# aleflabo/HypAD

Hardware: AMD Instinct MI355X
Metric: training windows/sec (seq_len=100) (higher is better)
Workload: dtype f32; 1 GPU; configs[1]: univariate synthetic (sine+noise+jump), hyperbolic=True, batch=64, window=100, latent=20, 1916 windows/signal, 1 signal(s) per GPU; step = 1 epoch = 29 x (5 critic_x + 5 critic_z + 1 decoder) iterations; signals_per_gpu=1, launch=hipGraph replay of the captured epoch, rccl_world_size=1

## Files before the change

### hypad_amd/csrc/train_common.h

```cpp
#pragma once
#include <hip/hip_runtime.h>

#include "../../include/hypad.h"
#include "critic_valu.h"
#include "nets.h"

namespace hypad {
namespace train {

constexpr int THREADS = 256;
constexpr int TB = 512;

struct CritWs {
  int in_right, act[4], left[5], dm[4], partial, total;
};
HD CritWs crit_ws(int B, int in_dim, int L, int nh) {
  CritWs w; int o = 0;
  w.in_right = o; o += pad4(3 * B * in_dim);
  for (int i = 0; i < 4; ++i) { w.act[i] = o; if (i < nh) o += pad4(3 * B * L); }
  for (int i = 0; i < 5; ++i) { w.left[i] = o; if (i < nh) o += pad4(3 * B * L); else if (i == nh) o += pad4(3 * B); }
  for (int i = 0; i < 4; ++i) { w.dm[i] = o; if (i < nh) o += pad4(B * L); }
  w.partial = o; o += pad4((B / 16) * 4);
  w.total = o;
  return w;
}
struct GenWs {
  int xg, enc_g, enc_g2, enc_h, zcat, a0, g0, h0d, mask, g1, h1, ecat, u, du, ballpart, dpre2, dg1, dg0, da0, dzenc, dgenc, partial, adamc, total;
};
HD GenWs gen_ws(int B, int S, int L) {
  GenWs w; int o = 0;
  w.xg = o; o += pad4(2 * B * S);
  w.enc_g = o; o += pad4(B * 8 * ENC_H);
  w.enc_g2 = o; o += pad4(B * 8 * ENC_H);
  w.enc_h = o; o += pad4(2 * B * 2 * ENC_H);
  w.zcat = o; o += pad4(2 * B * L);
  w.a0 = o; o += pad4(2 * B * DEC_D1);
  w.g0 = o; o += pad4(2 * B * 8 * DEC_H);
  w.h0d = o; o += pad4(2 * B * 2 * DEC_H);
  w.mask = o; o += pad4(2 * B * 2 * DEC_H);
  w.g1 = o; o += pad4(2 * B * 8 * DEC_H);
  w.h1 = o; o += pad4(2 * B * 2 * DEC_H);
  w.ecat = o; o += pad4(3 * B * S);
  w.u = o; o += pad4(3 * B * S);
  w.du = o; o += pad4(3 * B * S);
  w.ballpart = o; o += pad4(2 * (B / 16) * S);
  w.dpre2 = o; o += pad4(2 * B * S);
  w.dg1 = o; o += pad4(2 * B * 6 * DEC_H);
  w.dg0 = o; o += pad4(2 * B * 6 * DEC_H);
  w.da0 = o; o += pad4(2 * B * DEC_D1);
  w.dzenc = o; o += pad4(2 * B * L);
  w.dgenc = o; o += pad4(2 * B * 6 * ENC_H);
  w.partial = o; o += pad4((B / 16) * 4);
  w.adamc = o; o += 4;
  w.total = o;
  return w;
}
inline int64_t ws_cz_offset(const hypad_dims& d) { return crit_ws(d.batch, d.signal_shape, d.latent_dim, 4).total; }
inline int64_t ws_pack_offset(const hypad_dims& d) {
  int64_t a = ws_cz_offset(d) + crit_ws(d.batch, d.latent_dim, d.latent_dim, 2).total;
  int64_t c = gen_ws(d.batch, d.signal_shape, d.latent_dim).total;
  return ((a > c ? a : c) + 63) & ~(int64_t)63;
}
constexpr int DW_ITEM_WORDS = 32, DW_ITEM_CAP = 2048;
inline int64_t ws_items_offset(const hypad_dims& d) {
  return (ws_pack_offset(d) + gen_pack(d.signal_shape, d.latent_dim, d.hyperbolic).total + 63) & ~(int64_t)63;
}
inline int64_t ws_floats_per_signal(const hypad_dims& d) {
  return ws_items_offset(d) + (int64_t)DW_ITEM_WORDS * DW_ITEM_CAP;
}

struct IterArgs {
  int S, L, B, hyperbolic;
  hypad_nets P, M, V;
  int pe, pd, pcx, pcz;
  int32_t* counters;
  const float* x; int64_t x_sig_stride; int64_t x_ld; const int32_t* row_index;
  const float* z; const float* alpha;
  int drop_mode;
  const float* masks; int64_t mask_sig_stride;
  uint64_t seed;
  float* losses; int64_t loss_sig_stride;
  float* ws; int64_t ws_sig_stride;
  int64_t pk_off;
  float lr, b1, b2, eps, wd; int stabilize; int riemannian;
  int opt;
  int tick_owner;
  int sig0;
  int step_add;
  int rng_sig0;
  int64_t ri_sig_stride;
  int guard;
  long long* stamps;
};
#if HYPAD_DIAG
#define GEN_STAMP(k) do { if (a.stamps && (threadIdx.x & 63) == 0 && blockIdx.x == 0 && blockIdx.y == 0) a.stamps[(blockIdx.z * 48 + (k)) * 8 + (threadIdx.x >> 6)] = (long long)__builtin_amdgcn_s_memtime(); } while (0)
#else
#define GEN_STAMP(k) do { } while (0)
#endif

struct LdsPlan {
  int xs, zs, bufA, bufB, crit, small, wst, cparams, total, ldS, bufFloats;
  int stage;
};
constexpr int LDS_LIMIT_FLOATS = 160 * 1024 / 4;
HD LdsPlan lds_plan(int S, int rows_lstm, int rows_head, int critic_floats, int crit_scratch = CRITIC_LDS_FLOATS) {
  LdsPlan p;
  p.ldS = lds_stride(S);
  int a = rows_lstm * (6 * DEC_H + 4), b = rows_head * p.ldS;
  p.bufFloats = a > b ? a : b;
  int o = 0;
  p.xs = o; o += 16 * p.ldS;
  p.zs = o; o += 32 * LP;
  p.bufA = o; o += p.bufFloats;
  p.bufB = o; o += p.bufFloats;
  p.crit = o; o += crit_scratch;
  p.small = o; o += 3 * 16 * LP + 64;
  p.wst = o; o += (TB / 64) * WSTAGE_FLOATS;
  p.cparams = o;
  p.stage = (o + critic_floats <= LDS_LIMIT_FLOATS) ? 1 : 0;
  if (p.stage) o += critic_floats;
  p.total = o;
  return p;
}

__device__ __forceinline__ DropSrc drop_src(const IterArgs& a, int sig, const float* ptr, uint32_t stream, uint32_t tick, float p) {
  DropSrc s;
  s.mode = a.drop_mode; s.ptr = ptr; s.batch = a.B; s.seed = a.seed; s.tick = tick; s.stream = stream; s.sig = (uint32_t)(sig + a.rng_sig0); s.p = p;
  return s;
// ... 101 lines not shown
```

### hypad_amd/csrc/train_iters.hip

```cpp
#include <hip/hip_runtime.h>

#include <cstdlib>
#include <type_traits>

#include <vector>

#include "../../include/hypad.h"
#include "critic_mfma.h"
#include "train_common.h"

using namespace hypad;
using namespace hypad::train;

namespace {

__device__ __forceinline__ void critic_three_passes(const IterArgs& a, int sig, int tile, uint32_t tick, const float* real, int ldr,
                                                    const float* fake, int ldf, float* inter, int ldi, float* gbuf, int ldgb,
                                                    const float* P, const CriticLayout& cl, const CriticBatchLds& cb, float* ws,
                                                    const CritWs& cw, int mask_real, int mask_fake, int mask_inter, float* red) {
  const int L = a.L, B = a.B, nh = cl.nh, in_dim = cl.in_dim, LQ = cb.LQ;
  const int g0 = tile * 16;
  const float* mbase = a.masks ? a.masks + sig * a.mask_sig_stride : nullptr;
  const int64_t mblk = (int64_t)nh * B * L;
  const int midx[3] = {mask_real, mask_fake, mask_inter};
// ... 194 lines not shown
  const int a = 16 * (6 * DEC_H + 4), b = rows_head * p.ldS;
  const int bufFloats = a > b ? a : b;
  int o = 0;
  p.hb = o; o += (role == 1 && hyper) ? 16 * p.ldS : 0;
  p.xs = o; o += role >= 1 ? 16 * p.ldS : 0;
  p.zs = o; o += 32 * LP;
  p.bufA = o; o += bufFloats;
  p.bufB = o; o += bufFloats;
  p.small = o; o += 3 * 16 * LP + 64;
  p.cw = o; o += cp.total;
  p.ct = o; o += critic_tile_floats(cp, role == 0 ? 4 : 2);
  p.total = o;
  return p;
}

template <int SC, int LC, int BC, bool WSC1 = false>
__device__ __forceinline__ void gen_role_z(const IterArgs& a, float* smem) {
  const int S = SC ? SC : a.S, L = LC ? LC : a.L, B = BC ? BC : a.B;
  const int sig = blockIdx.y + a.sig0, tile = blockIdx.x >> 3;
  const GenLds lp = gen_lds(S, L, a.hyperbolic, 2);
  const int ldS = lp.ldS;
  const GenWs gw = gen_ws(B, S, L);
  float* ws = a.ws + sig * a.ws_sig_stride;
  const float* pk = ws + a.pk_off;
  const GenPack gp = gen_pack(S, L, a.hyperbolic);
  float* xs = smem + lp.xs; float* zs = smem + lp.zs; float* bufA = smem + lp.bufA; float* bufB = smem + lp.bufB;
  float* dzc = smem + lp.small;
  float* cw = smem + lp.cw; float* ct = smem + lp.ct;
  const uint32_t tick = (uint32_t)a.counters[3] + (uint32_t)(a.step_add > 0 ? a.step_add : 0);
  const int g0 = tile * 16;
  const float* mbase = a.masks ? a.masks + sig * a.mask_sig_stride : nullptr;
  const CriticLayout clz = cz_layout(L);
  const CriticPad cpz = critic_pad(L, L, 2);
  tile_load_rows(xs, ldS, a.x + sig * a.x_sig_stride, a.x_ld, a.row_index ? a.row_index + (int64_t)sig * a.ri_sig_stride : nullptr, g0, 16, S, 16);
  const LstmPre pre_enc = lstm_layer_prefetch<WSC1>(pk + gp.enc_g[0], pk + gp.enc_g[1], ENC_H, S);
  stage_critic_padded(cw, a.P.cz + (int64_t)sig * a.pcz, clz, L, cpz);
  __syncthreads();
  tile_store(ws + gw.xg + (int64_t)(B + g0) * S, S, xs, ldS, 16, S, 16);
  float* zin = zs + 16 * LP;
  float* gates = ws + gw.enc_g2 + (int64_t)g0 * 8 * ENC_H;
  encoder_fwd_tile_packed<true, WSC1>(xs, ldS, S, L, pk, gp, bufA, ENC_LDG, bufB, ENC_LDH, zin, gates,
                                ws + gw.enc_h + (int64_t)(B + g0) * 2 * ENC_H, 16, pre_enc);
  const PackedPre pre_edt = gemm_nt_prefetch<WSC1>(pk + gp.enc_d_t, L, 2 * ENC_H);
  const DropSrc dz = drop_src(a, sig, mbase, RS_DROP_CRITIC + 8 * 0, tick, clz.p_drop);
  const float sum_crit = critic_tile_fwd_bwd(zin, LP, cw, clz, L, cpz, ct, -1.f / B, [&](int li, int r, int c) { return dz.get4(li, g0 + r, c, L); },
                                             [&](int li, int r, int c) { return dz.get(li, g0 + r, c, L); }, dzc, LP);
  tile_store(ws + gw.dzenc + (int64_t)(B + g0) * L, L, dzc, LP, 16, L, 16);
  float* dP = bufA;
  {
    LstmCellBwdEpi epi{gates, ENC_H, dP, ENC_LDG, 16, 16, nullptr, 0, ws + gw.dgenc + (int64_t)(B + g0) * 6 * ENC_H, {}, {}, {}, {}, {}};
    gemm_nt_packed_epi<1, true, decltype(epi), WSC1>(dzc, LP, L, 2 * ENC_H, pk + gp.enc_d_t, nullptr, 0, pre_edt, epi);
  }
  float* part_out = ws + gw.partial + tile * 4;
  if (threadIdx.x == 0) part_out[2] = sum_crit;
  if (tile == 0 && blockIdx.y == 0 && threadIdx.x == 0) {
    const int step = a.counters[a.opt] + 1 + (a.step_add > 0 ? a.step_add : 0);
    if (a.step_add < 0) a.counters[a.opt] = step;
    const AdamCoef c0 = adam_coef(a.lr, a.b1, a.b2, a.eps, a.wd, a.riemannian, a.stabilize, step);
    float* ac = a.ws + (int64_t)a.sig0 * a.ws_sig_stride + gw.adamc;
    ac[0] = c0.bc1; ac[1] = c0.bc2; ac[2] = c0.sqrt_bc2;
  }
}

static_assert(TB == 512, "gen_body deals rows over 8 waves");
template <bool HYPER, int SC, int LC, int BC, bool WSC1 = false>
__device__ __forceinline__ void gen_body(const IterArgs& a, float* smem) {
  const int S = SC ? SC : a.S, L = LC ? LC : a.L, B = BC ? BC : a.B;
  const int sig = blockIdx.y + a.sig0, tile = blockIdx.x >> 3, role = blockIdx.z;
  __builtin_amdgcn_s_setprio(2);
  if (role == 2) { gen_role_z<SC, LC, BC, WSC1>(a, smem); return; }
  const GenLds lp = gen_lds(S, L, HYPER ? 1 : 0, role);
  const int ldS = lp.ldS;
  const EncLayout el = enc_layout(S, L);
  const DecLayout dl = dec_layout(S, L, HYPER ? 1 : 0);
  const GenWs gw = gen_ws(B, S, L);
  const float* PE = a.P.enc + (int64_t)sig * a.pe;
  const float* PD = a.P.dec + (int64_t)sig * a.pd;
  float* ws = a.ws + sig * a.ws_sig_stride;
  const float* pk = ws + a.pk_off;
  const GenPack gp = gen_pack(S, L, HYPER ? 1 : 0);
  float* xs = smem + lp.xs; float* zs = smem + lp.zs; float* bufA = smem + lp.bufA; float* bufB = smem + lp.bufB;
  float* small = smem + lp.small;
  float* red = small + 3 * 16 * LP;
  float* cw = smem + lp.cw; float* ct = smem + lp.ct;
  float* Ein = (HYPER && role == 1) ? smem + lp.hb : bufA;
  const uint32_t tick = (uint32_t)a.counters[3] + (uint32_t)(a.step_add > 0 ? a.step_add : 0);
  const int g0 = tile * 16;
  const int pass = role;
  const int64_t prow0 = (int64_t)pass * B + g0;
  const float* mbase = a.masks ? a.masks + sig * a.mask_sig_stride : nullptr;
  const int64_t BL = (int64_t)B * L;
  const int lane = threadIdx.x & 63, wave = wave_id(), nw = blockDim.x >> 6;
  float sum_crit = 0.f, sum_aux = 0.f;
  constexpr int ldH = 2 * DEC_H + 4, ldG = 6 * DEC_H + 4, ldA0 = 52;
  GEN_STAMP(0);
  float* zin;
  PackedPre pre_d1;
  if (role == 0) {
    pre_d1 = gemm_nt_prefetch<WSC1>(pk + gp.d1, L, DEC_D1);
    const CriticLayout clx = cx_layout(S, L);
    stage_critic_padded(cw, a.P.cx + (int64_t)sig * a.pcx, clx, L, critic_pad(S, L, 4));
    load_z(a, sig, tile, tick, zs);
    zin = zs;
    __syncthreads();
  } else {
    GEN_STAMP(14);
    tile_load_rows(xs, ldS, a.x + sig * a.x_sig_stride, a.x_ld, a.row_index ? a.row_index + (int64_t)sig * a.ri_sig_stride : nullptr, g0, 16, S, 16);
    const LstmPre pre_enc = lstm_layer_prefetch<WSC1>(pk + gp.enc_g[0], pk + gp.enc_g[1], ENC_H, S);
    GEN_STAMP(15);
    GEN_STAMP(12);
    __syncthreads();
    GEN_STAMP(13);
    tile_store(ws + gw.xg + (int64_t)g0 * S, S, xs, ldS, 16, S, 16);
    if (HYPER) tile_store(ws + gw.ecat + (int64_t)(2 * B + g0) * S, S, xs, ldS, 16, S, 16);
    zin = zs + 16 * LP;
    encoder_fwd_tile_packed<true, WSC1>(xs, ldS, S, L, pk, gp, bufA, ENC_LDG, bufB, ENC_LDH, zin,
                                  ws + gw.enc_g + (int64_t)g0 * 8 * ENC_H, ws + gw.enc_h + (int64_t)g0 * 2 * ENC_H, 16, pre_enc);
    GEN_STAMP(1);
    pre_d1 = gemm_nt_prefetch<WSC1>(pk + gp.d1, L, DEC_D1);
  }
  GEN_STAMP(2);
  tile_store(ws + gw.zcat + prow0 * L, L, zin, LP, 16, L, 16);
  DecSave sv;
  sv.ps = 16;
  sv.a0 = ws + gw.a0 + prow0 * DEC_D1;
// ... 29 lines not shown
        for (int e = 0; e < EPL; ++e) { u_keep[e] = u.v[e]; hb_keep[e] = hb.v[e]; }
        row_store(bufB + r * ldS, head_row(u, hb), S, lane);
      }
    });
    __syncthreads();
  }
  float* R = HYPER ? bufB : bufA;
  float* dR = HYPER ? bufA : bufB;
  GEN_STAMP(4);
  if (role == 0) {
    const CriticLayout clx = cx_layout(S, L);
    const DropSrc dx = drop_src(a, sig, mbase ? mbase + 2 * BL : nullptr, RS_DROP_CRITIC + 8 * 1, tick, clx.p_drop);
    sum_crit = critic_tile_fwd_bwd(R, ldS, cw, clx, L, critic_pad(S, L, 4), ct, -1.f / B,
                                   [&](int li, int r, int c) { return dx.get4(li, g0 + r, c, L); },
                                   [&](int li, int r, int c) { return dx.get(li, g0 + r, c, L); }, dR, ldS);
  }
  GEN_STAMP(5);
  if (HYPER) {
    if (role == 1) {
      float part = 0.f;
      if (wave < 4) {
        epl16_dispatch(S, [&](auto tag) {
          using R16 = RowT<16, decltype(tag)::value>;
          const int r = wave * 4 + (lane >> 4);
          R16 du, dv;
          const float d = rowdist_row_bwd(row_load<R16>(R + r * ldS, S, lane), row_load<R16>(R + (16 + r) * ldS, S, lane), 10.f / B, du, dv);
          row_store(dR + r * ldS, du, S, lane);
          row_store(dR + (16 + r) * ldS, dv, S, lane);
          const float d0 = __int_as_float(__builtin_amdgcn_readlane(__float_as_int(d), 0)), d1 = __int_as_float(__builtin_amdgcn_readlane(__float_as_int(d), 16));
          const float d2 = __int_as_float(__builtin_amdgcn_readlane(__float_as_int(d), 32)), d3 = __int_as_float(__builtin_amdgcn_readlane(__float_as_int(d), 48));
          part = (d0 + d1) + (d2 + d3);
        });
      }
      if (lane == 0) red[16 + wave] = part;
      __syncthreads();
      for (int w = 0; w < nw; ++w) sum_aux += red[16 + w];
    }
    GEN_STAMP(23);
    const PackedPre pre_ht = gemm_nt_prefetch<WSC1>(pk + gp.head_t, S, S);
    epl16_dispatch(S, [&](auto tag) {
      constexpr int EPL = decltype(tag)::value;
      using R16 = RowT<16, EPL>;
      const int r = wave * 4 + (lane >> 4);
      if (wave * 4 < hrows) {
        R16 du, db, u, hb;
#pragma unroll
        for (int e = 0; e < EPL; ++e) { u.v[e] = u_keep[e]; hb.v[e] = hb_keep[e]; }
        head_row_bwd(u, hb, row_load<R16>(dR + r * ldS, S, lane), du, db);
        row_store(dR + r * ldS, du, S, lane);
        row_store(ws + gw.du + (prow0 + prow(r, B)) * S, du, S, lane);
#pragma unroll
        for (int e = 0; e < R16::EPL; ++e) {
          float v = db.v[e];
          v += __shfl_xor(v, 16, 64);
          v += __shfl_xor(v, 32, 64);
          db.v[e] = v;
        }
        if (lane < 16) row_store(R + wave * ldS, db, S, lane);
      }
    });
    __syncthreads();
    GEN_STAMP(24);
    for (int c = threadIdx.x; c < S; c += blockDim.x) {
      float s = 0.f;
      for (int w = 0; w < hrows / 4; ++w) s += R[w * ldS + c];
      ws[gw.ballpart + ((int64_t)role * (B / 16) + tile) * S + c] = s;
    }
    __syncthreads();
    GEN_STAMP(25);
    {
      struct TanhBwdEpi {
        float* Ys; int ldy; const float* E; int ldE; float* gout; float e[4]; int vo;
        __device__ __forceinline__ void prefetch(int n, int q, bool ok) {
          vo = (4 * q * ldE + (ok ? n : 0)) * 4;
          const GBuf eb(E);
#pragma unroll
          for (int r = 0; r < 4; ++r) e[r] = ok ? eb.ld(vo, r * ldE * 4) : 0.f;
        }
        __device__ __forceinline__ void emit(int, int r, int row, int n, float v) {
          const float o = v * (1.f - e[r] * e[r]);
          Ys[row * ldy + n] = o; GBuf(gout).st(o, vo, r * ldE * 4);
        }
      } epi{R, ldS, ws + gw.ecat + prow0 * S, S, ws + gw.dpre2 + prow0 * S, {}, 0};
      gemm_nt_packed_epi<1, true, decltype(epi), WSC1>(dR, ldS, S, S, pk + gp.head_t, nullptr, 0, pre_ht, epi);
    }
    __syncthreads();
    GEN_STAMP(26);
  } else {
    if (role == 1) {
      float part = 0.f;
      tile_for(16, S, [&](int r, int c) {
        const float diff = R[r * ldS + c] - xs[r * ldS + c];
        part += diff * diff;
        dR[r * ldS + c] = 20.f * diff / ((float)B * (float)S);
      });
      sum_aux = block_sum(part, red);
      __syncthreads();
    }
    tile_for(16, S, [&](int r, int c) {
      const float e = R[r * ldS + c];
      dR[r * ldS + c] *= 1.f - e * e;
// ... 20 lines not shown
    LstmCellBwdEpi epi{ws + gw.g0 + prow0 * 8 * DEC_H, DEC_H, X, ldG, 16, 16,
                       a.drop_mode != 0 ? ws + gw.mask + prow0 * 2 * DEC_H : nullptr, 2 * DEC_H, ws + gw.dg0 + prow0 * 6 * DEC_H, {}, {}, {}, {}, {}};
    gemm_nt_packed_epi<1, true, decltype(epi), WSC1>(Y, ldG, 6 * DEC_H, 2 * DEC_H, pk + gp.l_t[1], nullptr, 0, pre_l1t, epi);
  }
  GEN_STAMP(35);
  __syncthreads();
  GEN_STAMP(36);
  GEN_STAMP(8);
  GEN_STAMP(37);
  PackedPre pre_d1t{};
  if (role == 1) pre_d1t = gemm_nt_prefetch<WSC1>(pk + gp.d1_t, DEC_D1, L);
  GEN_STAMP(38);
  gemm_nt_packed<1, true, ActIdentity, WSC1>(X, ldG, 6 * DEC_H, DEC_D1, pk + gp.l_t[0], nullptr, Y, ldA0, 0, 0, pre_l0t, ActIdentity{}, nullptr, 0,
                          ws + gw.da0 + prow0 * DEC_D1, DEC_D1);
  GEN_STAMP(39);
  __syncthreads();
  GEN_STAMP(9);
  float* part_out = ws + gw.partial + tile * 4;
  if (role == 0) {
    if (threadIdx.x == 0) part_out[1] = sum_crit;
    GEN_STAMP(11);
    return;
  }
  const PackedPre pre_edt = gemm_nt_prefetch<WSC1>(pk + gp.enc_d_t, L, 2 * ENC_H);
  gemm_nt_packed<1, true, ActIdentity, WSC1>(Y, ldA0, DEC_D1, L, pk + gp.d1_t, nullptr, X, LP, 0, 0, pre_d1t, ActIdentity{}, nullptr, 0,
                          ws + gw.dzenc + (int64_t)g0 * L, L);
  __syncthreads();
  GEN_STAMP(10);
  {
    LstmCellBwdEpi epi{ws + gw.enc_g + (int64_t)g0 * 8 * ENC_H, ENC_H, Y, ENC_LDG, 16, 16, nullptr, 0,
                       ws + gw.dgenc + (int64_t)g0 * 6 * ENC_H, {}, {}, {}, {}, {}};
    gemm_nt_packed_epi<1, true, decltype(epi), WSC1>(X, LP, L, 2 * ENC_H, pk + gp.enc_d_t, nullptr, 0, pre_edt, epi);
  }
  if (threadIdx.x == 0) part_out[0] = sum_aux;
  GEN_STAMP(11);
}

__global__ __launch_bounds__(TB) void cx_pass_kernel(IterArgs a) {
  extern __shared__ __attribute__((aligned(16))) float smem[];
  cx_pass_body(a, smem);
}
__global__ __launch_bounds__(TB) void cz_pass_kernel(IterArgs a) {
  extern __shared__ __attribute__((aligned(16))) float smem[];
  cz_pass_body(a, smem);
}
__global__ __launch_bounds__(TB) void critic_pass_pair_kernel(IterArgs ax, IterArgs az) {
  extern __shared__ __attribute__((aligned(16))) float smem[];
  if (blockIdx.z == 0) cx_pass_body(ax, smem); else cz_pass_body(az, smem);
}
template <bool IS_X>
__global__ __launch_bounds__(TB) void critic_gp_kernel(IterArgs a) {
  extern __shared__ __attribute__((aligned(16))) float smem[];
  gp_body<IS_X>(a, smem);
}
__global__ __launch_bounds__(TB) void critic_gp_pair_kernel(IterArgs ax, IterArgs az) {
  extern __shared__ __attribute__((aligned(16))) float smem[];
  if (blockIdx.z == 0) gp_body<true>(ax, smem); else gp_body<false>(az, smem);
}
template <bool HYPER, int SC, int LC, int BC>
__global__ __launch_bounds__(TB) void gen_kernel(IterArgs a) {
  extern __shared__ __attribute__((aligned(16))) float smem[];
  if (a.guard && a.counters[4] != 0) return;
  if ((blockIdx.x & 7) != ((blockIdx.y + a.sig0 + (blockIdx.z == 2 ? 1 : 0)) & 7)) return;
  gen_body<HYPER, SC, LC, BC, true>(a, smem);
}

enum DwKind : int { DW_WEIGHT = 0, DW_BIAS = 1, DW_DECAY = 2, DW_BALL = 3 };
// ... 30 lines not shown
  if (net == HYPAD_NET_ENCODER) {
    const EncLayout el = enc_layout(S, L);
    for (int d = 0; d < 2; ++d) {
      const int w = el.dir[d].w_ih, wg = w + 2 * ENC_H * S;
      if (p_off == w || p_off == wg) { r.fwd = gp.enc_g[d]; r.fwd_kg = (S + 15) >> 4; r.nbase = p_off == w ? 0 : ENC_H; r.gate_H = ENC_H; }
      const int b = el.dir[d].b_ih;
      if (p_off == b || p_off == b + 2 * ENC_H) { r.bsum = gp.enc_gb[d]; r.nbase = p_off == b ? 0 : ENC_H; r.gate_H = ENC_H; }
    }
    if (p_off == el.dense_w) { r.fwd = gp.enc_d; r.fwd_kg = (2 * ENC_H + 15) >> 4; r.bwd = gp.enc_d_t; r.bwd_ng = (L + 15) >> 4; }
    if (p_off == el.dense_b) r.bsum = gp.enc_db;
  } else if (net == HYPAD_NET_DECODER) {
    const DecLayout dl = dec_layout(S, L, hyper);
    if (p_off == dl.d1_w) { r.fwd = gp.d1; r.fwd_kg = (L + 15) >> 4; r.bwd = gp.d1_t; r.bwd_ng = (DEC_D1 + 15) >> 4; }
    if (p_off == dl.d1_b) r.bsum = gp.d1b;
    for (int l = 0; l < 2; ++l) {
      const int in = l == 0 ? DEC_D1 : 2 * DEC_H;
      for (int d = 0; d < 2; ++d) {
        const int w = dl.l[l][d].w_ih, wg = w + 2 * DEC_H * in;
        if (p_off == w || p_off == wg) {
          r.fwd = gp.l_g[l][d]; r.fwd_kg = (in + 15) >> 4; r.nbase = p_off == w ? 0 : DEC_H; r.gate_H = DEC_H;
          r.bwd = gp.l_t[l]; r.bwd_ng = (6 * DEC_H) >> 4; r.mbase = d * 3 * DEC_H;
        }
        const int b = dl.l[l][d].b_ih;
        if (p_off == b || p_off == b + 2 * DEC_H) { r.bsum = gp.l_gb[l][d]; r.nbase = p_off == b ? 0 : DEC_H; r.gate_H = DEC_H; }
      }
    }
    if (p_off == dl.d2_w) { r.fwd = gp.d2; r.fwd_kg = (2 * DEC_H + 15) >> 4; r.bwd = gp.d2_t; r.bwd_ng = (S + 15) >> 4; }
    if (p_off == dl.d2_b) r.bsum = gp.d2b;
    if (hyper && p_off == dl.head_w) { r.fwd = gp.head; r.fwd_kg = (S + 15) >> 4; r.bwd = gp.head_t; r.bwd_ng = (S + 15) >> 4; }
  }
  return r;
}

constexpr int DW_KS_MANY = 16;
template <class Table, int SC = 0, int LC = 0, int BC = 0, int KS = 48>
__device__ __forceinline__ void dw_adam_body(const IterArgs& a, const Table& tab, const int bx = (int)blockIdx.x) {
  const int S_ = SC ? SC : a.S, L_ = LC ? LC : a.L, B_ = BC ? BC : a.B;
  const int sig = blockIdx.y + a.sig0;
  const int lane = threadIdx.x & 63, wave = wave_id();
  const int j = lane & 15, q = lane >> 4;
  float* ws = a.ws + sig * a.ws_sig_stride;
  const int item = bx * (THREADS / 64) + wave;
  const int di = (tab.block_desc[bx >> 2] >> (8 * (bx & 3))) & 0xff;
  const DwDesc d = tab.d[di];
  const int step = a.counters[a.opt] + (a.step_add >= 0 ? a.step_add + 1 : 0);
  const float* ac = a.ws + (tab.finalize == 1 ? (int64_t)a.sig0 * a.ws_sig_stride + gen_ws(B_, S_, L_).adamc : 0);
  const float ac0 = ac[0], ac1 = ac[1], ac2 = ac[2];
  AdamCoef co;
  if (tab.finalize == 1) {
    co.lr = a.lr; co.b1 = a.b1; co.b2 = a.b2; co.eps = a.eps; co.wd = a.wd; co.riemannian = a.riemannian; co.stabilize = a.stabilize;
    co.step = step; co.bc1 = ac0; co.bc2 = ac1; co.sqrt_bc2 = ac2;
  } else {
    co = adam_coef(a.lr, a.b1, a.b2, a.eps, a.wd, a.riemannian, a.stabilize, step);
  }
  const int64_t arena = d.net == HYPAD_NET_ENCODER ? a.pe : d.net == HYPAD_NET_DECODER ? a.pd : d.net == HYPAD_NET_CRITIC_X ? a.pcx : a.pcz;
  auto pick = [&](const hypad_nets& n) __attribute__((always_inline)) {
    float* base = d.net == HYPAD_NET_ENCODER ? n.enc : d.net == HYPAD_NET_DECODER ? n.dec : d.net == HYPAD_NET_CRITIC_X ? n.cx : n.cz;
    return base + sig * arena;
  };
  if (item < tab.total_items) {
    const int local = item - d.begin;
    float* P = pick(a.P); float* M = pick(a.M); float* V = pick(a.V);
    if (d.kind == DW_WEIGHT && local < ((d.nrows + 15) >> 4) * ((d.ncols + 15) >> 4)) {
      const int tk = (d.ncols + 15) >> 4;
      const int n0 = (local / tk) * 16, k0 = (local % tk) * 16;
      const int nj = n0 + j < d.nrows ? n0 + j : d.nrows - 1, kj = k0 + j < d.ncols ? k0 + j : d.ncols - 1;
// ... 73 lines not shown
        int64_t o = d.p_off + n;
        float p = P[o], m = M[o], v = V[o];
        adam_update(p, m, v, g, co);
        P[o] = p; M[o] = m; V[o] = v;
        float bs = p;
        if (d.p_off2 >= 0) {
          o = d.p_off2 + n;
          p = P[o]; m = M[o]; v = V[o];
          adam_update(p, m, v, g, co);
          P[o] = p; M[o] = m; V[o] = v;
          bs += p;
        }
        if (tab.finalize == 1) {
          const ShadowRef sh = shadow_ref(d.net, d.p_off, S_, L_, a.hyperbolic);
          if (sh.bsum >= 0) {
            int nf = sh.nbase + n;
            if (sh.gate_H > 0) { const int x = nf / sh.gate_H; nf = x * ((sh.gate_H + 15) & ~15) + nf - x * sh.gate_H; }
            ws[a.pk_off + sh.bsum + nf] = bs;
          }
        }
      }
    } else if (d.kind == DW_DECAY) {
#pragma unroll
      for (int e = 0; e < 4; ++e) {
        const int n = local * 256 + e * 64 + lane;
        if (n < d.nrows) {
          const int64_t o = d.p_off + n;
          float p = P[o], m = M[o], v = V[o];
          adam_update(p, m, v, 0.f, co);
          P[o] = p; M[o] = m; V[o] = v;
        }
      }
    } else if (d.kind == DW_BALL && local == 0) {
      const float* left = ws + d.left_off;
      RowVec g;
#pragma unroll
      for (int e = 0; e < MAX_EPL; ++e) g.v[e] = 0.f;
      for (int r0 = 0; r0 < d.red_rows; r0 += 8) {
        float t[8][MAX_EPL];
#pragma unroll
        for (int u = 0; u < 8; ++u) {
          const int r = r0 + u < d.red_rows ? r0 + u : d.red_rows - 1;
#pragma unroll
          for (int e = 0; e < MAX_EPL; ++e) {
            const int c = lane + 64 * e;
            t[u][e] = c < d.nrows ? left[(int64_t)r * d.left_ld + c] : 0.f;
          }
        }
#pragma unroll
        for (int u = 0; u < 8; ++u)
#pragma unroll
          for (int e = 0; e < MAX_EPL; ++e) g.v[e] += r0 + u < d.red_rows ? t[u][e] : 0.f;
      }
      radam_ball_wave(P + d.p_off, M + d.p_off, V + d.p_off, g, d.nrows, lane, co);
    }
  }
#if HYPAD_DIAG
  if (a.stamps && tab.finalize == 1 && blockIdx.y == 0 && lane == 0 && item < 1024) {
    a.stamps[3 * 48 * 8 + 64 + 2 * item] = (long long)__builtin_amdgcn_s_memrealtime();
    a.stamps[3 * 48 * 8 + 64 + 2 * item + 1] = item < tab.total_items ? d.kind * 1000 + d.net * 100 + (d.red_rows >> 4) : -1;
  }
#endif
  if (bx == 0 && threadIdx.x == 0) {
    if (tab.finalize == 1) {
      const GenWs gw = gen_ws(B_, S_, L_);
      float aux = 0.f, fx = 0.f, fz = 0.f;
      for (int t = 0; t < B_ / 16; ++t) {
        const float* part = ws + gw.partial + t * 4;
        aux += part[0]; fx += part[1]; fz += part[2];
      }
      aux = a.hyperbolic ? aux / a.B : aux / ((float)a.B * (float)a.S);
      float* lo = a.losses + sig * a.loss_sig_stride;
      lo[0] = 10.f * aux - fx / a.B - fz / a.B;
      lo[1] = aux; lo[2] = fx / a.B; lo[3] = fz / a.B;
    }
    if (blockIdx.y == 0 && a.tick_owner && a.step_add < 0) a.counters[3] += 1;
  }
}
struct DwItem {
  int32_t kind;
  int32_t net;
  int32_t n0, k0;
  int32_t nrows, ncols, p_off, p_ld, p_off2;
  int32_t left_off, left_ld, right_off, right_ld, red_rows;
  int32_t fwd, fwd_kg, nbase, bwd, bwd_ng, mbase, bsum, gate_H;
  int32_t table_sig;
  int32_t pad[9];
};
__host__ __device__ inline int32_t dw_table_sig(int total_items, int S, int L, int hyper, int n_desc) {
  uint32_t h = 0x9E3779B9u * (uint32_t)(total_items + 1);
  h ^= (uint32_t)S << 20; h ^= (uint32_t)L << 10; h ^= (uint32_t)n_desc << 2; h ^= (uint32_t)(hyper ? 1 : 0);
  return (int32_t)(h | 0x40000000u);
}
static_assert(sizeof(DwItem) == 4 * DW_ITEM_WORDS, "DwItem is DW_ITEM_WORDS words");
__global__ __launch_bounds__(256) void dw_items_kernel(DwTable tab, DwItem* __restrict__ out, int S, int L, int hyper) {
  const int item = blockIdx.x * 256 + threadIdx.x;
  if (item >= DW_ITEM_CAP) return;
  DwItem it{};
  it.kind = -1;
  it.table_sig = dw_table_sig(tab.total_items, S, L, hyper, tab.n);
  if (item < tab.total_items) {
    const int bx = item >> 2;
// ... 137 lines not shown
      g += __shfl_xor(g, 16, WAVE);
      g += __shfl_xor(g, 32, WAVE);
      if (own) {
        float p = p1_, m = m1_, v = v1_;
        adam_update(p, m, v, g, co);
        P[o1] = p; M[o1] = m; V[o1] = v;
        float bs = p;
        if (d.p_off2 >= 0) {
          p = p2_; m = m2_; v = v2_;
          adam_update(p, m, v, g, co);
          P[o2] = p; M[o2] = m; V[o2] = v;
          bs += p;
        }
        if (d.bsum >= 0) {
          int nf = d.nbase + n;
          if (d.gate_H > 0) { const int x = nf / d.gate_H; nf = x * ((d.gate_H + 15) & ~15) + nf - x * d.gate_H; }
          ws[a.pk_off + d.bsum + nf] = bs;
        }
      }
    } else if (d.kind == DW_DECAY) {
#pragma unroll
      for (int e = 0; e < 4; ++e) {
        const int n = d.n0 + e * 64 + lane;
        if (n < d.nrows) {
          const int64_t o = d.p_off + n;
          float p = P[o], m = M[o], v = V[o];
          adam_update(p, m, v, 0.f, co);
          P[o] = p; M[o] = m; V[o] = v;
        }
      }
    } else if (d.kind == DW_BALL) {
      const float* left = ws + d.left_off;
      const RowVec Pr = row_load(P + d.p_off, d.nrows, lane), Mr = row_load(M + d.p_off, d.nrows, lane), Vr = row_load(V + d.p_off, d.nrows, lane);
      RowVec g;
#pragma unroll
      for (int e = 0; e < MAX_EPL; ++e) g.v[e] = 0.f;
      for (int r0 = 0; r0 < d.red_rows; r0 += 8) {
        float t[8][MAX_EPL];
#pragma unroll
        for (int u = 0; u < 8; ++u) {
          const int r = r0 + u < d.red_rows ? r0 + u : d.red_rows - 1;
#pragma unroll
          for (int e = 0; e < MAX_EPL; ++e) {
            const int c = lane + 64 * e;
            t[u][e] = c < d.nrows ? left[(int64_t)r * d.left_ld + c] : 0.f;
          }
        }
#pragma unroll
        for (int u = 0; u < 8; ++u)
#pragma unroll
          for (int e = 0; e < MAX_EPL; ++e) g.v[e] += r0 + u < d.red_rows ? t[u][e] : 0.f;
      }
      radam_ball_wave(P + d.p_off, M + d.p_off, V + d.p_off, Pr, Mr, Vr, g, d.nrows, lane, co);
    }
  }
#if HYPAD_DIAG
  if (a.stamps && model == 0 && lane == 0 && item < 1024) {
    a.stamps[3 * 48 * 8 + 64 + 2 * item] = (long long)__builtin_amdgcn_s_memrealtime();
    a.stamps[3 * 48 * 8 + 64 + 2 * item + 1] = item < total_items && d.kind >= 0 ? d.kind * 1000 + d.net * 100 + (d.red_rows >> 4) : -1;
  }
#endif
  if (bx == 0 && threadIdx.x == 0) {
    const GenWs gw = gen_ws(B_, S_, L_);
    float aux = 0.f, fx = 0.f, fz = 0.f;
    for (int t = 0; t < B_ / 16; ++t) {
      const float* part = ws + gw.partial + t * 4;
      aux += part[0]; fx += part[1]; fz += part[2];
    }
    aux = a.hyperbolic ? aux / a.B : aux / ((float)a.B * (float)a.S);
    float* lo = a.losses + sig * a.loss_sig_stride;
    lo[0] = 10.f * aux - fx / a.B - fz / a.B;
    lo[1] = aux; lo[2] = fx / a.B; lo[3] = fz / a.B;
    if (model == 0 && a.tick_owner && a.step_add < 0) a.counters[3] += 1;
  }
}
template <int SC, int LC, int BC, int KS, bool COLOC = false>
__global__ __launch_bounds__(THREADS) void dw_adam_kernel(IterArgs a, const DwItem* __restrict__ items, int total_items, int chunk, int32_t table_sig) {
  if (a.guard && a.counters[4] != 0) return;
  if constexpr (COLOC) {
    const int blocks = (total_items + THREADS / 64 - 1) / (THREADS / 64);
    const int t = (int)(blockIdx.x >> 3), model = (t / blocks) * 8 + (int)(blockIdx.x & 7);
    if (model >= chunk) return;
    dw_adam_items_body<SC, LC, BC, KS>(a, items, total_items, t % blocks, table_sig, 0, model);
  } else {
    dw_adam_items_body<SC, LC, BC, KS>(a, items, total_items, (int)blockIdx.x, table_sig, chunk);
  }
}
__global__ __launch_bounds__(THREADS) void dw_adam_small_kernel(IterArgs a, DwTableS tab) { dw_adam_body(a, tab); }
__global__ __launch_bounds__(THREADS) void dw_adam_pair_kernel(IterArgs ax, DwTableS tx, IterArgs az, DwTableS tz) {
  if (blockIdx.z == 0) dw_adam_body(ax, tx); else dw_adam_body(az, tz);
}

template <class Table>
struct TableBuilder {
  Table t;
  bool overflow = false;
  TableBuilder() { t.n = 0; t.total_items = 0; t.finalize = 0; for (int i = 0; i < Table::blk / 4; ++i) t.block_desc[i] = 0; }
  void push(DwDesc d, int items) {
    if (items <= 0) return;
    const int start = (t.total_items + 3) & ~3;
    const int b0 = start / 4, b1 = (start + items + 3) / 4;
    if (t.n >= Table::cap || b1 > Table::blk) { overflow = true; return; }
    d.begin = start;
    for (int b = b0; b < b1; ++b) t.block_desc[b >> 2] |= (uint32_t)t.n << (8 * (b & 3));
    t.d[t.n++] = d;
    t.total_items = start + items;
  }
  Table done() { if (overflow) t.n = -1; return t; }
  void weight(int net, int p_off, int p_ld, int nrows, int ncols, int left_off, int left_ld, int right_off, int right_ld, int red) {
    DwDesc d{};
    d.kind = DW_WEIGHT; d.net = (int16_t)net; d.p_off = p_off; d.p_ld = p_ld; d.nrows = nrows; d.ncols = ncols;
    d.left_off = left_off; d.left_ld = left_ld; d.right_off = right_off; d.right_ld = right_ld; d.red_rows = red; d.p_off2 = -1;
    push(d, ((nrows + 15) / 16) * ((ncols + 15) / 16));
  }
  void bias(int net, int p_off, int p_off2, int n, int left_off, int left_ld, int red) {
    DwDesc d{};
    d.kind = DW_BIAS; d.net = (int16_t)net; d.p_off = p_off; d.p_off2 = p_off2; d.nrows = n; d.ncols = 1;
    d.left_off = left_off; d.left_ld = left_ld; d.red_rows = red;
    push(d, (n + 15) / 16);
  }
  bool skip_decay = false;
  void decay(int net, int p_off, int n) {
    if (skip_decay) return;
    DwDesc d{};
    d.kind = DW_DECAY; d.net = (int16_t)net; d.p_off = p_off; d.nrows = n; d.p_off2 = -1;
    push(d, (n + 255) / 256);
  }
  void ball(int net, int p_off, int n, int left_off, int left_ld, int red) {
    DwDesc d{};
    d.kind = DW_BALL; d.net = (int16_t)net; d.p_off = p_off; d.nrows = n; d.left_off = left_off; d.left_ld = left_ld;
    d.red_rows = red; d.p_off2 = -1;
    push(d, 1);
  }
  void lstm_dir(int net, const LstmDir& ld, int H, int K, int left_off, int left_ld, int c0, int right_off, int right_ld, int red,
                bool decay_too) {
    weight(net, ld.w_ih, K, H, K, left_off + c0, left_ld, right_off, right_ld, red);
    weight(net, ld.w_ih + 2 * H * K, K, 2 * H, K, left_off + c0 + H, left_ld, right_off, right_ld, red);
    bias(net, ld.b_ih, ld.b_hh, H, left_off + c0, left_ld, red);
    bias(net, ld.b_ih + 2 * H, ld.b_hh + 2 * H, 2 * H, left_off + c0 + H, left_ld, red);
    if (decay_too) {
      decay(net, ld.w_ih + H * K, H * K);
      decay(net, ld.w_hh, 4 * H * H);
      decay(net, ld.b_ih + H, H);
      decay(net, ld.b_hh + H, H);
    }
  }
};

DwTableS critic_table(int net, const CriticLayout& cl, const CritWs& cw, int B, int L) {
  TableBuilder<DwTableS> tb;
  for (int li = 0; li <= cl.nh; ++li) {
    int k = li == 0 ? cl.in_dim : L, n = li == cl.nh ? 1 : L;
    int right = li == 0 ? cw.in_right : cw.act[li - 1];
    tb.weight(net, cl.w[li], k, n, k, cw.left[li], n, right, k, 3 * B);
    tb.bias(net, cl.b[li], -1, n, cw.left[li], n, 2 * B);
  }
  return tb.done();
}

struct DecayTable { int n, total; int net[24], off[24], len[24], begin[24]; };
DecayTable decay_table(const hypad_dims& dm) {
  DecayTable t{};
  const int S = dm.signal_shape, L = dm.latent_dim;
// ... 33 lines not shown
    __syncthreads();
    const int n = nsteps - s0 < 64 ? nsteps - s0 : 64;
    for (int k = 0; k < n; ++k) {
      co.bc1 = bc[2 * k]; co.bc2 = bc[2 * k + 1];
      adam_update(p, m, v, 0.f, co);
    }
  }
  if (live) { *P = p; *M = m; *V = v; }
}

DwTable gen_table(const hypad_dims& dm, bool with_decay = true) {
  const int B = dm.batch, S = dm.signal_shape, L = dm.latent_dim;
  const bool hyp = dm.hyperbolic != 0;
  const EncLayout el = enc_layout(S, L);
  const DecLayout dl = dec_layout(S, L, dm.hyperbolic);
  const GenWs gw = gen_ws(B, S, L);
  TableBuilder<DwTable> tb;
  tb.t.finalize = 1;
  tb.skip_decay = !with_decay;
  for (int d = 0; d < 2; ++d)
    tb.lstm_dir(HYPAD_NET_ENCODER, el.dir[d], ENC_H, S, gw.dgenc, 6 * ENC_H, d * 3 * ENC_H, gw.xg, S, 2 * B, hyp);
  tb.weight(HYPAD_NET_ENCODER, el.dense_w, 2 * ENC_H, L, 2 * ENC_H, gw.dzenc, L, gw.enc_h, 2 * ENC_H, 2 * B);
  tb.bias(HYPAD_NET_ENCODER, el.dense_b, -1, L, gw.dzenc, L, 2 * B);
  tb.weight(HYPAD_NET_DECODER, dl.d1_w, L, DEC_D1, L, gw.da0, DEC_D1, gw.zcat, L, 2 * B);
  tb.bias(HYPAD_NET_DECODER, dl.d1_b, -1, DEC_D1, gw.da0, DEC_D1, 2 * B);
  for (int d = 0; d < 2; ++d) {
    tb.lstm_dir(HYPAD_NET_DECODER, dl.l[0][d], DEC_H, DEC_D1, gw.dg0, 6 * DEC_H, d * 3 * DEC_H, gw.a0, DEC_D1, 2 * B, hyp);
    tb.lstm_dir(HYPAD_NET_DECODER, dl.l[1][d], DEC_H, 2 * DEC_H, gw.dg1, 6 * DEC_H, d * 3 * DEC_H, gw.h0d, 2 * DEC_H, 2 * B, hyp);
  }
  tb.weight(HYPAD_NET_DECODER, dl.d2_w, 2 * DEC_H, S, 2 * DEC_H, gw.dpre2, S, gw.h1, 2 * DEC_H, 2 * B);
  tb.bias(HYPAD_NET_DECODER, dl.d2_b, -1, S, gw.dpre2, S, 2 * B);
  if (hyp) {
    tb.weight(HYPAD_NET_DECODER, dl.head_w, S, S, S, gw.du, S, gw.ecat, S, 3 * B);
    tb.ball(HYPAD_NET_DECODER, dl.head_b, S, gw.ballpart, S, 2 * (B / 16));
  }
  return tb.done();
}

bool critic_launches_fit(int S, int L) {
  const int cxf = cx_layout(S, L).total, czf = cz_layout(L).total, scratch = critic_batch_lds_floats(48, L);
  const int f[4] = {lds_plan(S, 16, 16, cxf, scratch).total, lds_plan(S, 16, 16, czf, scratch).total, gp_lds_floats(S, cxf),
                    gp_lds_floats(L, czf)};
  for (int v : f)
    if ((size_t)v * sizeof(float) > 160 * 1024) return false;
  return true;
}

int check_dims(const hypad_dims* d) {
  if (!d || d->signal_shape <= 0 || d->latent_dim <= 0 || d->batch <= 0 || d->n_signals <= 0 || d->first_signal < 0) return HYPAD_EINVAL;
  if (d->batch % 16 != 0) return HYPAD_EINVAL;
  if (d->signal_shape > MAX_S || d->latent_dim > MAX_L) return HYPAD_EUNSUPPORTED;
  if (!critic_launches_fit(d->signal_shape, d->latent_dim)) return HYPAD_EUNSUPPORTED;
  if (gen_table(*d).n < 0) return HYPAD_EUNSUPPORTED;
  const CriticLayout cls[2] = {cx_layout(d->signal_shape, d->latent_dim), cz_layout(d->latent_dim)};
  for (const CriticLayout& cl : cls)
    for (int li = 0; li <= cl.nh; ++li)
      if (cl.wof(li) != cl.w[li] || cl.bof(li) != cl.b[li]) return HYPAD_EUNSUPPORTED;
  return HYPAD_OK;
}

struct PackDesc {
  int kind;
  int net;
  int dst, nout, kred;
  int src0, src1, ld, H;
};
struct PackTable { int n; int max_units; PackDesc d[32]; };
// ... 706 lines not shown
```

Baseline: 729,500 windows/s.

## Write per-wave ball-bias and aux partials to workspace, reduce in optimizer

The generator body no longer does a block-wide LDS reduction and an extra __syncthreads for the hyperbolic head-bias gradient and the aux loss. Each wave now writes its own partial row to a larger global ballpart or auxpart buffer. The dw/Adam stage sums these rows with a new ball_grad_rows helper that keeps the original grouped summation order, and the loss finalizer sums the aux partials. This trims a barrier and a serial reduction from the latency-critical generator path, in exchange for more rows to read in the optimizer's single-wave ball update.

```diff
diff --git a/hypad_amd/csrc/train_common.h b/hypad_amd/csrc/train_common.h
--- a/hypad_amd/csrc/train_common.h
+++ b/hypad_amd/csrc/train_common.h
@@ -25,8 +25,9 @@
   return w;
 }
 struct GenWs {
-  int xg, enc_g, enc_g2, enc_h, zcat, a0, g0, h0d, mask, g1, h1, ecat, u, du, ballpart, dpre2, dg1, dg0, da0, dzenc, dgenc, partial, adamc, total;
-};
+  int xg, enc_g, enc_g2, enc_h, zcat, a0, g0, h0d, mask, g1, h1, ecat, u, du, ballpart, dpre2, dg1, dg0, da0, dzenc, dgenc, partial, auxpart, adamc, total;
+};
+HD int ball_row(int role, int tile, int wave, int ntile) { return role == 0 ? tile * 4 + wave : ntile * 4 + tile * 8 + wave; }
 HD GenWs gen_ws(int B, int S, int L) {
   GenWs w; int o = 0;
   w.xg = o; o += pad4(2 * B * S);
@@ -43,7 +44,7 @@
   w.ecat = o; o += pad4(3 * B * S);
   w.u = o; o += pad4(3 * B * S);
   w.du = o; o += pad4(3 * B * S);
-  w.ballpart = o; o += pad4(2 * (B / 16) * S);
+  w.ballpart = o; o += pad4(12 * (B / 16) * S);
   w.dpre2 = o; o += pad4(2 * B * S);
   w.dg1 = o; o += pad4(2 * B * 6 * DEC_H);
   w.dg0 = o; o += pad4(2 * B * 6 * DEC_H);
@@ -51,6 +52,7 @@
   w.dzenc = o; o += pad4(2 * B * L);
   w.dgenc = o; o += pad4(2 * B * 6 * ENC_H);
   w.partial = o; o += pad4((B / 16) * 4);
+  w.auxpart = o; o += pad4((B / 16) * 4);
   w.adamc = o; o += 4;
   w.total = o;
   return w;
@@ -93,7 +95,7 @@
   long long* stamps;
 };
 #if HYPAD_DIAG
-#define GEN_STAMP(k) do { if (a.stamps && (threadIdx.x & 63) == 0 && blockIdx.x == 0 && blockIdx.y == 0) a.stamps[(blockIdx.z * 48 + (k)) * 8 + (threadIdx.x >> 6)] = (long long)__builtin_amdgcn_s_memtime(); } while (0)
+#define GEN_STAMP(k) do { if (a.stamps && (threadIdx.x & 63) == 0 && (blockIdx.x >> 3) == 0 && blockIdx.y == 0) a.stamps[(blockIdx.z * 48 + (k)) * 8 + (threadIdx.x >> 6)] = (long long)__builtin_amdgcn_s_memtime(); } while (0)
 #else
 #define GEN_STAMP(k) do { } while (0)
 #endif
diff --git a/hypad_amd/csrc/train_iters.hip b/hypad_amd/csrc/train_iters.hip
--- a/hypad_amd/csrc/train_iters.hip
+++ b/hypad_amd/csrc/train_iters.hip
@@ -250,6 +250,7 @@
   const float* mbase = a.masks ? a.masks + sig * a.mask_sig_stride : nullptr;
   const CriticLayout clz = cz_layout(L);
   const CriticPad cpz = critic_pad(L, L, 2);
+  GEN_STAMP(0);
   tile_load_rows(xs, ldS, a.x + sig * a.x_sig_stride, a.x_ld, a.row_index ? a.row_index + (int64_t)sig * a.ri_sig_stride : nullptr, g0, 16, S, 16);
   const LstmPre pre_enc = lstm_layer_prefetch<WSC1>(pk + gp.enc_g[0], pk + gp.enc_g[1], ENC_H, S);
   stage_critic_padded(cw, a.P.cz + (int64_t)sig * a.pcz, clz, L, cpz);
@@ -278,6 +279,7 @@
     float* ac = a.ws + (int64_t)a.sig0 * a.ws_sig_stride + gw.adamc;
     ac[0] = c0.bc1; ac[1] = c0.bc2; ac[2] = c0.sqrt_bc2;
   }
+  GEN_STAMP(11);
 }
 
 static_assert(TB == 512, "gen_body deals rows over 8 waves");
@@ -308,7 +310,7 @@
   const int64_t prow0 = (int64_t)pass * B + g0;
   const float* mbase = a.masks ? a.masks + sig * a.mask_sig_stride : nullptr;
   const int64_t BL = (int64_t)B * L;
-  const int lane = threadIdx.x & 63, wave = wave_id(), nw = blockDim.x >> 6;
+  const int lane = threadIdx.x & 63, wave = wave_id();
   float sum_crit = 0.f, sum_aux = 0.f;
   constexpr int ldH = 2 * DEC_H + 4, ldG = 6 * DEC_H + 4, ldA0 = 52;
   GEN_STAMP(0);
@@ -404,9 +406,8 @@
           part = (d0 + d1) + (d2 + d3);
         });
       }
-      if (lane == 0) red[16 + wave] = part;
+      if (lane == 0 && wave < 4) ws[gw.auxpart + tile * 4 + wave] = part;
       __syncthreads();
-      for (int w = 0; w < nw; ++w) sum_aux += red[16 + w];
     }
     GEN_STAMP(23);
     const PackedPre pre_ht = gemm_nt_prefetch<WSC1>(pk + gp.head_t, S, S);
@@ -428,17 +429,11 @@
           v += __shfl_xor(v, 32, 64);
           db.v[e] = v;
         }
-        if (lane < 16) row_store(R + wave * ldS, db, S, lane);
+        if (lane < 16) row_store(ws + gw.ballpart + (int64_t)ball_row(role, tile, wave, B / 16) * S, db, S, lane);
       }
     });
     __syncthreads();
     GEN_STAMP(24);
-    for (int c = threadIdx.x; c < S; c += blockDim.x) {
-      float s = 0.f;
-      for (int w = 0; w < hrows / 4; ++w) s += R[w * ldS + c];
-      ws[gw.ballpart + ((int64_t)role * (B / 16) + tile) * S + c] = s;
-    }
-    __syncthreads();
     GEN_STAMP(25);
     {
       struct TanhBwdEpi {
@@ -525,7 +520,7 @@
                        ws + gw.dgenc + (int64_t)g0 * 6 * ENC_H, {}, {}, {}, {}, {}};
     gemm_nt_packed_epi<1, true, decltype(epi), WSC1>(X, LP, L, 2 * ENC_H, pk + gp.enc_d_t, nullptr, 0, pre_edt, epi);
   }
-  if (threadIdx.x == 0) part_out[0] = sum_aux;
+  if (!HYPER && threadIdx.x == 0) part_out[0] = sum_aux;
   GEN_STAMP(11);
 }
 
@@ -622,6 +617,45 @@
   return r;
 }
 
+template <int NB, int EPL>
+__device__ __forceinline__ RowVec ball_grad_rows(const float* __restrict__ left, int ld, int n, int rows, int rows4, int lane) {
+  RowVec g;
+  float s[EPL];
+#pragma unroll
+  for (int e = 0; e < MAX_EPL; ++e) g.v[e] = 0.f;
+#pragma unroll
+  for (int e = 0; e < EPL; ++e) s[e] = 0.f;
+  const GBuf lb(left);
+  int vo[EPL];
+#pragma unroll
+  for (int e = 0; e < EPL; ++e) vo[e] = (lane + 64 * e < n ? lane + 64 * e : n - 1) * 4;
+#pragma unroll 1
+  for (int r0 = 0; r0 < rows; r0 += NB) {
+    float t[NB][EPL];
+#pragma unroll
+    for (int u = 0; u < NB; ++u) {
+      const int r = r0 + u < rows ? r0 + u : rows - 1;
+#pragma unroll
+      for (int e = 0; e < EPL; ++e) t[u][e] = lb.ld(vo[e], r * ld * 4);
+    }
+#pragma unroll
+    for (int u = 0; u < NB; ++u) {
+      const int r = r0 + u;
+      if (r < rows) {
+#pragma unroll
+        for (int e = 0; e < EPL; ++e) s[e] += t[u][e];
+        if (r < rows4 ? (r & 3) == 3 : ((r - rows4) & 7) == 7) {
+#pragma unroll
+          for (int e = 0; e < EPL; ++e) { g.v[e] += s[e]; s[e] = 0.f; }
+        }
+      }
+    }
+  }
+#pragma unroll
+  for (int e = 0; e < EPL; ++e) g.v[e] = lane + 64 * e < n ? g.v[e] : 0.f;
+  return g;
+}
+template <int KS, int EPL> constexpr int ball_rows_in_flight() { return KS >= 48 ? (144 / EPL < KS ? 144 / EPL : KS) : 32 / EPL; }
 constexpr int DW_KS_MANY = 16;
 template <class Table, int SC = 0, int LC = 0, int BC = 0, int KS = 48>
 __device__ __forceinline__ void dw_adam_body(const IterArgs& a, const Table& tab, const int bx = (int)blockIdx.x) {
@@ -761,26 +795,7 @@
         }
       }
     } else if (d.kind == DW_BALL && local == 0) {
-      const float* left = ws + d.left_off;
-      RowVec g;
-#pragma unroll
-      for (int e = 0; e < MAX_EPL; ++e) g.v[e] = 0.f;
-      for (int r0 = 0; r0 < d.red_rows; r0 += 8) {
-        float t[8][MAX_EPL];
-#pragma unroll
-        for (int u = 0; u < 8; ++u) {
-          const int r = r0 + u < d.red_rows ? r0 + u : d.red_rows - 1;
-#pragma unroll
-          for (int e = 0; e < MAX_EPL; ++e) {
-            const int c = lane + 64 * e;
-            t[u][e] = c < d.nrows ? left[(int64_t)r * d.left_ld + c] : 0.f;
-          }
-        }
-#pragma unroll
-        for (int u = 0; u < 8; ++u)
-#pragma unroll
-          for (int e = 0; e < MAX_EPL; ++e) g.v[e] += r0 + u < d.red_rows ? t[u][e] : 0.f;
-      }
+      const RowVec g = ball_grad_rows<8, MAX_EPL>(ws + d.left_off, d.left_ld, d.nrows, d.red_rows, d.ncols, lane);
       radam_ball_wave(P + d.p_off, M + d.p_off, V + d.p_off, g, d.nrows, lane, co);
     }
   }
@@ -796,7 +811,13 @@
       float aux = 0.f, fx = 0.f, fz = 0.f;
       for (int t = 0; t < B_ / 16; ++t) {
         const float* part = ws + gw.partial + t * 4;
-        aux += part[0]; fx += part[1]; fz += part[2];
+        fx += part[1]; fz += part[2];
+        if (a.hyperbolic) {
+          const float* wp = ws + gw.auxpart + t * 4;
+          float at = 0.f;
+          for (int w = 0; w < 4; ++w) at += wp[w];
+          aux += at;
+        } else aux += part[0];
       }
       aux = a.hyperbolic ? aux / a.B : aux / ((float)a.B * (float)a.S);
       float* lo = a.losses + sig * a.loss_sig_stride;
@@ -1000,25 +1021,9 @@
     } else if (d.kind == DW_BALL) {
       const float* left = ws + d.left_off;
       const RowVec Pr = row_load(P + d.p_off, d.nrows, lane), Mr = row_load(M + d.p_off, d.nrows, lane), Vr = row_load(V + d.p_off, d.nrows, lane);
-      RowVec g;
-#pragma unroll
-      for (int e = 0; e < MAX_EPL; ++e) g.v[e] = 0.f;
-      for (int r0 = 0; r0 < d.red_rows; r0 += 8) {
-        float t[8][MAX_EPL];
-#pragma unroll
-        for (int u = 0; u < 8; ++u) {
-          const int r = r0 + u < d.red_rows ? r0 + u : d.red_rows - 1;
-#pragma unroll
-          for (int e = 0; e < MAX_EPL; ++e) {
-            const int c = lane + 64 * e;
-            t[u][e] = c < d.nrows ? left[(int64_t)r * d.left_ld + c] : 0.f;
-          }
-        }
-#pragma unroll
-        for (int u = 0; u < 8; ++u)
-#pragma unroll
-          for (int e = 0; e < MAX_EPL; ++e) g.v[e] += r0 + u < d.red_rows ? t[u][e] : 0.f;
-      }
+      constexpr int EPL = SC ? (SC + 63) / 64 : MAX_EPL;
+      const RowVec g = ball_grad_rows<ball_rows_in_flight<KS, EPL>(), EPL>(left, SC ? SC : d.left_ld, SC ? SC : d.nrows, BC ? 12 * (BC / 16) : d.red_rows,
+                                                                          BC ? 4 * (BC / 16) : d.ncols, lane);
       radam_ball_wave(P + d.p_off, M + d.p_off, V + d.p_off, Pr, Mr, Vr, g, d.nrows, lane, co);
     }
   }
@@ -1033,7 +1038,13 @@
     float aux = 0.f, fx = 0.f, fz = 0.f;
     for (int t = 0; t < B_ / 16; ++t) {
       const float* part = ws + gw.partial + t * 4;
-      aux += part[0]; fx += part[1]; fz += part[2];
+      fx += part[1]; fz += part[2];
+      if (a.hyperbolic) {
+        const float* wp = ws + gw.auxpart + t * 4;
+        float at = 0.f;
+        for (int w = 0; w < 4; ++w) at += wp[w];
+        aux += at;
+      } else aux += part[0];
     }
     aux = a.hyperbolic ? aux / a.B : aux / ((float)a.B * (float)a.S);
     float* lo = a.losses + sig * a.loss_sig_stride;
@@ -1094,9 +1105,9 @@
     d.kind = DW_DECAY; d.net = (int16_t)net; d.p_off = p_off; d.nrows = n; d.p_off2 = -1;
     push(d, (n + 255) / 256);
   }
-  void ball(int net, int p_off, int n, int left_off, int left_ld, int red) {
+  void ball(int net, int p_off, int n, int left_off, int left_ld, int red, int red4) {
     DwDesc d{};
-    d.kind = DW_BALL; d.net = (int16_t)net; d.p_off = p_off; d.nrows = n; d.left_off = left_off; d.left_ld = left_ld;
+    d.kind = DW_BALL; d.net = (int16_t)net; d.p_off = p_off; d.nrows = n; d.ncols = red4; d.left_off = left_off; d.left_ld = left_ld;
     d.red_rows = red; d.p_off2 = -1;
     push(d, 1);
   }
@@ -1196,7 +1207,7 @@
   tb.bias(HYPAD_NET_DECODER, dl.d2_b, -1, S, gw.dpre2, S, 2 * B);
   if (hyp) {
     tb.weight(HYPAD_NET_DECODER, dl.head_w, S, S, S, gw.du, S, gw.ecat, S, 3 * B);
-    tb.ball(HYPAD_NET_DECODER, dl.head_b, S, gw.ballpart, S, 2 * (B / 16));
+    tb.ball(HYPAD_NET_DECODER, dl.head_b, S, gw.ballpart, S, 12 * (B / 16), 4 * (B / 16));
   }
   return tb.done();
 }
```

New measurement: 731,900 windows/s (median of 6 runs). No clear change (+0.3%).
